# Hengle/AkariRender-1

Hardware: AMD Instinct MI355X
Metric: Msamples/sec (whole node), 10M-tri scene 1080p 1024spp, 1/2/4/8 MI355X (higher is better)
Workload: dtype f32; 1 GPU; C3 synthetic triangle soup (SURVEY.md §8d); triangles=10000002, width=1920, height=1080, spp=1025, max_depth=5, tile=64, parallelism=tile-split x1, bvh_leaf=4, builder=sbvh, form=k_path, ordered_fetch=True

## Files before the change

### akarirender-1_amd/akari_amd/capi.py

```python
from __future__ import annotations

import ctypes as C
import os
from pathlib import Path

import numpy as np

PKG_DIR = Path(__file__).resolve().parent.parent
PRODUCT_LIB = PKG_DIR / "libakr_hip.so"
EXPERIMENT_LIB_DIR = PKG_DIR.parent / "tools" / "experiments" / "lib"
LIB_PATH = Path(os.environ.get("AKR_HIP_LIB", PRODUCT_LIB))
if LIB_PATH != PRODUCT_LIB and LIB_PATH.resolve().parent != EXPERIMENT_LIB_DIR.resolve():
    raise ImportError(f"AKR_HIP_LIB={LIB_PATH}: only tools/experiments/lib/*.so may replace the product library")
GEN_PATH = PKG_DIR / "libakr_scenegen.so"


class AkrError(RuntimeError):
    """A non-zero status from the C-ABI (the reference's AKR_ASSERT_THROW convention)."""


class Ray(C.Structure):
    _fields_ = [("o", C.c_float * 3), ("tmin", C.c_float), ("d", C.c_float * 3), ("tmax", C.c_float)]


# ... 152 lines not shown
    "akr_hip_import_accel": (C.c_int, [_P, _P, C.c_uint64, _P, C.c_uint64, C.c_int32]),
    "akr_bvh_validate": (C.c_int, [_P, C.c_uint64, _P, C.c_uint64, C.c_uint64, C.POINTER(C.c_int32)]),
    "akr_hip_accel_info": (C.c_int, [_P, C.POINTER(AccelInfo)]),
    "akr_hip_accel_export": (C.c_int, [_P, _P, C.c_uint64, _P, C.c_uint64]),
    "akr_hip_set_camera": (C.c_int, [_P, C.POINTER(Camera)]),
    "akr_hip_set_lens": (C.c_int, [_P, C.c_float, C.c_float]),
    "akr_hip_lens": (C.c_int, [_P, C.POINTER(C.c_float), C.POINTER(C.c_float), C.POINTER(C.c_int32)]),
    "akr_hip_trace": (C.c_int, [_P, _P, C.c_uint64, _P, C.c_int]),
    "akr_hip_trace_device": (C.c_int, [_P, _P, C.c_uint64, _P, C.c_int, _P]),
    "akr_hip_render": (C.c_int, [_P, C.POINTER(PtParams), _P, C.c_int32, _P, _P]),
    "akr_hip_render_ao": (C.c_int, [_P, C.POINTER(AoParams), _P, C.c_int32, _P, _P]),
    "akr_hip_ray_steps": (C.c_int, [_P, _P, C.c_uint64]),
    "akr_hip_render_device": (C.c_int, [_P, C.POINTER(PtParams), _P, C.c_int32, _P, _P, _P,
                                        C.POINTER(C.c_uint64)]),
    "akr_hip_kernel_stats": (C.c_int, [_P, _P, C.c_int32, C.POINTER(C.c_int32)]),
    "akr_hip_trace_counts": (C.c_int, [_P, C.POINTER(TraceCounts)]),
    "akr_hip_path_profile": (C.c_int, [_P, C.POINTER(C.c_uint64), C.c_int32]),
    "akr_hip_reset_stats": (C.c_int, [_P]),
    "akr_hip_render_info": (C.c_int, [_P, C.POINTER(C.c_int32), C.POINTER(C.c_int32)]),
    "akr_hip_synchronize": (C.c_int, [_P]),
    "akr_hip_render_form": (C.c_int, [_P, C.POINTER(C.c_int32), C.POINTER(C.c_int32)]),
    "akr_hip_render_shading": (C.c_int, [_P, C.POINTER(C.c_int32)]),
    "akr_hip_render_form_inputs": (C.c_int, [_P, C.POINTER(C.c_int64), C.POINTER(C.c_int64), C.POINTER(C.c_int64)]),
    "akr_hip_pixel_probe": (C.c_int, [_P, _P, C.c_uint64]),
    "akr_bvh_host_build": (C.c_int, [_P, C.c_uint64, _P, C.c_uint64, C.POINTER(BuildParams), C.POINTER(_P),
                                     C.POINTER(AccelInfo)]),
    "akr_bvh_host_nodes": (_P, [_P]),
    "akr_bvh_host_tris": (_P, [_P]),
    "akr_bvh_host_free": (None, [_P]),
    "akr_hip_render_node": (C.c_int, [C.POINTER(_P), C.c_int32, C.POINTER(PtParams), _P, C.c_int32, _P, _P]),
    "akr_bvh_host_wide": (C.c_int, [_P, C.POINTER(C.c_uint64), C.POINTER(C.c_uint64), C.POINTER(C.c_uint32)]),
    "akr_bvh_host_wide_nodes": (_P, [_P]),
    "akr_bvh_host_wide_leaves": (_P, [_P]),
    "akr_hip_render_continue": (C.c_int, [_P, C.c_int32, _P, _P]),
    "akr_hip_render_continue_device": (C.c_int, [_P, C.c_int32, _P, _P, _P, C.POINTER(C.c_uint64)]),
    "akr_hip_render_state_info": (C.c_int, [_P, C.POINTER(RenderStateInfo)]),
    "akr_hip_render_state_export": (C.c_int, [_P, _P, _P, C.c_uint64]),
    "akr_hip_render_state_import": (C.c_int, [_P, C.POINTER(PtParams), _P, C.c_int32, _P, _P, C.c_uint64]),
    "akr_hip_render_continue_masked": (C.c_int, [_P, C.c_int32, _P, C.c_uint64, _P, _P]),
    "akr_hip_render_continue_masked_device": (C.c_int, [_P, C.c_int32, _P, C.c_uint64, _P, _P, _P,
                                                        C.POINTER(C.c_uint64)]),
    "akr_hip_render_state_spp_range": (C.c_int, [_P, C.POINTER(C.c_int32), C.POINTER(C.c_int32)]),
    "akr_hip_render_adaptive": (C.c_int, [_P, C.POINTER(PtParams), C.POINTER(AdaptiveParams), _P, C.c_int32, _P, _P,
                                          C.POINTER(AdaptiveInfo)]),
    "akr_hip_render_adaptive_device": (C.c_int, [_P, C.POINTER(PtParams), C.POINTER(AdaptiveParams), _P, C.c_int32,
                                                 _P, _P, _P, C.POINTER(C.c_uint64), C.POINTER(AdaptiveInfo)]),
    "akr_hip_adaptive_begin": (C.c_int, [_P, C.POINTER(PtParams), C.POINTER(AdaptiveParams), _P, C.c_int32,
                                         C.POINTER(AdaptiveInfo), C.POINTER(C.c_int32)]),
    "akr_hip_adaptive_step": (C.c_int, [_P, C.POINTER(AdaptiveInfo), C.POINTER(C.c_int32)]),
    "akr_hip_adaptive_error": (C.c_int, [_P, _P, _P, C.c_uint64]),
    "akr_hip_render_features": (C.c_int, [_P, C.POINTER(FeatureParams), _P, C.c_int32, _P]),
    "akr_hip_render_features_device": (C.c_int, [_P, C.POINTER(FeatureParams), _P, C.c_int32, _P, _P,
                                                 C.POINTER(C.c_uint64)]),
    "akr_hip_denoise": (C.c_int, [_P, C.POINTER(DenoiseParams), C.c_int32, C.c_int32, _P, _P, _P, _P]),
    "akr_hip_denoise_device": (C.c_int, [_P, C.POINTER(DenoiseParams), C.c_int32, C.c_int32, _P, _P, _P, _P, _P]),
    "akr_hip_render_variance": (C.c_int, [_P, _P]),
    "akr_hip_render_variance_device": (C.c_int, [_P, _P, _P, C.POINTER(C.c_uint64)]),
    "akr_hip_denoise_guided": (C.c_int, [_P, C.POINTER(DenoiseGuidedParams), C.c_int32, C.c_int32, _P, _P, _P, _P, _P]),
    "akr_hip_denoise_guided_device": (C.c_int, [_P, C.POINTER(DenoiseGuidedParams), C.c_int32, C.c_int32, _P, _P, _P, _P,
                                                _P, _P]),
}

_lib = None


def load_library() -> C.CDLL:
# ... 24 lines not shown
    lib = load_library()
    v = np.ascontiguousarray(vertices, np.float32).reshape(-1)
    i = np.ascontiguousarray(indices, np.int32).reshape(-1)
    p = BuildParams(max_leaf_size, n_bins, traversal_cost, intersect_cost, n_threads, builder, spatial_budget,
                    wide_collapse)
    h = C.c_void_p()
    info = AccelInfo()
    st = lib.akr_bvh_host_build(_ptr(v), v.size // 3, _ptr(i), i.size // 3, C.byref(p), C.byref(h), C.byref(info))
    if st != 0:
        raise AkrError("akr_bvh_host_build failed (invalid indices or build error)")
    try:
        nodes = np.empty(info.n_nodes, NODE_DTYPE)
        tris = np.empty(info.n_tris, TRI_DTYPE)
        C.memmove(nodes.ctypes.data, lib.akr_bvh_host_nodes(h), nodes.nbytes)
        if tris.nbytes:
            C.memmove(tris.ctypes.data, lib.akr_bvh_host_tris(h), tris.nbytes)
        if wide:
            nn, nl, root = C.c_uint64(0), C.c_uint64(0), C.c_uint32(0)
            if lib.akr_bvh_host_wide(h, C.byref(nn), C.byref(nl), C.byref(root)) != 0:
                raise AkrError("akr_bvh_host_wide failed")
            wn = np.empty(nn.value, NODE4_DTYPE)
            lv = np.empty(nl.value, LEAF_DTYPE)
            if wn.nbytes:
                C.memmove(wn.ctypes.data, lib.akr_bvh_host_wide_nodes(h), wn.nbytes)
            if lv.nbytes:
                C.memmove(lv.ctypes.data, lib.akr_bvh_host_wide_leaves(h), lv.nbytes)
    finally:
        lib.akr_bvh_host_free(h)
    if wide:
        return nodes, tris, info, (wn, lv, root.value)
    return nodes, tris, info


def validate_bvh(nodes, tris, n_scene_tris):
    nodes = np.ascontiguousarray(nodes, NODE_DTYPE)
    tris = np.ascontiguousarray(tris, TRI_DTYPE)
    d = C.c_int32(0)
    if load_library().akr_bvh_validate(_ptr(nodes), nodes.shape[0], _ptr(tris), tris.shape[0], int(n_scene_tris),
                                       C.byref(d)) != 0:
        raise AkrError("malformed BVH")
    return d.value


def render_node(ctxs, spp, max_depth, tiles, width, height, ray_clamp=0.0, exact_cull=False, radiance=None,
                weight=None, mis=None):
    lib = load_library()
    if mis is not None:
        for c in ctxs:
            c.set_option("mis", 1 if mis else 0)
    if radiance is None:
        radiance = np.zeros((height, width, 3), np.float32)
    if weight is None:
        weight = np.zeros((height, width), np.float32)
    assert radiance.dtype == np.float32 and radiance.flags.c_contiguous and radiance.size == 3 * width * height
    assert weight.dtype == np.float32 and weight.flags.c_contiguous and weight.size == width * height
    arr = (Rect * max(1, len(tiles)))(*[Rect(*t) for t in tiles])
    hs = (C.c_void_p * len(ctxs))(*[c.h for c in ctxs])
    p = PtParams(int(spp), int(max_depth), float(ray_clamp), PT_EXACT_CULL if exact_cull else 0)
    if lib.akr_hip_render_node(hs, len(ctxs), C.byref(p), _arr_ptr(arr), len(tiles), _ptr(radiance),
                               _ptr(weight)) != 0:
        raise AkrError(lib.akr_hip_last_error(ctxs[0].h).decode() if ctxs else "no contexts")
    return radiance, weight


def _ptr(a: np.ndarray):
    return a.ctypes.data_as(C.c_void_p)
# ... 487 lines not shown
```

### akarirender-1_amd/csrc/akr_device.h

```cpp
#pragma once
#include <stddef.h>
#include <stdint.h>
#include <hip/hip_runtime.h>
#include "../../include/akr_hip.h"
#include "../../include/akr_bvh_format.h"
#include "akr_path_forms.h"

#if defined(__HIP_DEVICE_COMPILE__)
#define AKR_GLOBAL __attribute__((address_space(1)))
#else
#define AKR_GLOBAL
#endif

namespace akr {

constexpr int kBlock = 256;
#ifndef AKR_TRACE_BLOCK
#define AKR_TRACE_BLOCK 256
#endif
constexpr int kTraceBlock = AKR_TRACE_BLOCK;
#ifndef AKR_STACK_LDS
#define AKR_STACK_LDS 15
#endif
#ifndef AKR_REFILL_MIN
// ... 34 lines not shown

__host__ __device__ inline uint32_t shard_begin(uint32_t n, uint32_t k) {
    return (uint32_t)(((uint64_t)n * k) / kWorkShards);
}

struct LightDev {
    float v[9];
    float tc[6];
    int32_t color_img;
    float Le[3];
    float area_half;
    float lng[3];
    float sel_pdf;
};

struct MatDev {
    int32_t type, double_sided, first, second;
    float color[3];
    int32_t color_img;
    float rough;
    int32_t rough_img;
    float frac;
    int32_t frac_img;
};
static_assert(sizeof(LightDev) == 96, "LightDev: six float4");

struct ShadeTri {
    float4 a;
    float4 b;
    float4 c;
    float4 d;
    float4 e;
};

struct TexDev {
    int32_t type;
    float value[3];
    int32_t w, h;
    int64_t off;
};

struct SceneDev {
    const AKR_GLOBAL ShadeTri *tri;
    const AKR_GLOBAL float *texcoords;
    int32_t has_image_tex;
    const AKR_GLOBAL MatDev *mats;
    const AKR_GLOBAL TexDev *texs;
    const AKR_GLOBAL float *images;
    const AKR_GLOBAL LightDev *lights;
    const AKR_GLOBAL float *light_cdf;
    int32_t n_lights;
    int32_t n_mats;
};

struct CameraDev {
    float r2c[16];
    float c2w[16];
    int32_t width, height;
};

struct TraceCounters {
    unsigned long long rays, box, tri;
    unsigned long long slots_trav, slots_leaf, slots_tri;
    unsigned long long visits;
    unsigned long long deep;
    unsigned long long leaves;
// ... 228 lines not shown
```

### akarirender-1_amd/csrc/bvh_build.h

```cpp
#pragma once
#include <stdint.h>
#include <exception>
#include <thread>
#include <vector>
#include "../../include/akr_hip.h"
#include "../../include/akr_bvh_format.h"

namespace akr {

template <class F>
void run_on_threads(int n, F &&f) {
    std::vector<std::exception_ptr> err((size_t)(n > 0 ? n : 0));
    auto call = [&](int k) {
        try {
            f(k);
        } catch (...) {
            err[(size_t)k] = std::current_exception();
        }
    };
    std::vector<std::thread> ts;
    std::vector<int> inline_k;
    for (int k = 1; k < n; k++) {
        try {
            ts.emplace_back(call, k);
// ... 9 lines not shown
}

struct BvhInput {
    const float *vertices;
    const int32_t *indices;
    uint64_t n_tris;
};

struct BvhOutput {
    std::vector<akr_bvh_node> nodes;
    std::vector<akr_bvh_tri> tris;
    int max_depth = 0;
    int max_leaf = 0;
    double sah_cost = 0;
    double build_ms = 0;
};

void build_bvh(const BvhInput &in, const akr_build_params &params, BvhOutput &out);

#ifdef __HIPCC__
void build_lbvh_gpu(const BvhInput &in, BvhOutput &out, hipStream_t st);
#endif

struct Bvh4Output {
    std::vector<akr_bvh4_node> nodes;
    std::vector<akr_bvh_leaf> leaves;
    uint32_t root_ref = AKR_CHILD_EMPTY;
    int max_depth = 0;
    float max_abs = 0.0f;
};

void build_bvh4(const std::vector<akr_bvh_node> &bvh2, Bvh4Output &out, int n_threads = 0, int collapse = 0);

int validate_bvh2(const akr_bvh_node *nodes, uint64_t n_nodes, const akr_bvh_tri *tris, uint64_t n_tris,
                  uint64_t n_scene_tris, int &max_leaf);

uint32_t quantize_lo(float bound, float origin, float s);
uint32_t quantize_hi(float bound, float origin, float s);

}
```

### akarirender-1_amd/csrc/bvh_wide.cpp

```cpp
#include <atomic>
#include <cmath>
#include <exception>
#include <thread>
#include <cstring>
#include <stdexcept>
#include "bvh_build.h"

namespace akr {

static bool real_le(uint32_t q, float s, float origin, float bound) {
    const long double v = (long double)origin + (long double)q * (long double)s;
    const long double m = std::ldexp(1.0L, -60) * (std::fabs((long double)origin) + 255.0L * s + std::fabs((long double)bound));
    return v + m <= (long double)bound;
}

static bool real_ge(uint32_t q, float s, float origin, float bound) {
    const long double v = (long double)origin + (long double)q * (long double)s;
    const long double m = std::ldexp(1.0L, -60) * (std::fabs((long double)origin) + 255.0L * s + std::fabs((long double)bound));
    return v - m >= (long double)bound;
}

namespace {

inline float pow2f(int k) { return std::ldexp(1.0f, k); }
// ... 298 lines not shown
                build(tasks[i], depth_of[w], abs_of[w], 0xffffffffu, no_spawn);
        });
        for (int w = 0; w < n_threads; w++) {
            max_depth = std::max(max_depth, depth_of[w]);
            max_abs = std::max(max_abs, abs_of[w]);
        }
        out.max_depth = max_depth;
        out.max_abs = max_abs;
    }
};

}

uint32_t quantize_lo(float bound, float origin, float s) {
    double q = std::floor(((double)bound - (double)origin) / (double)s);
    q = std::min(255.0, std::max(0.0, q));
    uint32_t qi = (uint32_t)q;
    while (qi > 0 && (std::fmaf((float)qi, s, origin) > bound || !real_le(qi, s, origin, bound))) qi--;
    if (std::fmaf((float)qi, s, origin) > bound || (qi > 0 && !real_le(qi, s, origin, bound)))
        throw std::runtime_error("quantize_lo: bound below origin");
    return qi;
}

uint32_t quantize_hi(float bound, float origin, float s) {
    double q = std::ceil(((double)bound - (double)origin) / (double)s);
    q = std::min(255.0, std::max(0.0, q));
    uint32_t qi = (uint32_t)q;
    while (qi < 255 && (std::fmaf((float)qi, s, origin) < bound || !real_ge(qi, s, origin, bound))) qi++;
    if (std::fmaf((float)qi, s, origin) < bound || !real_ge(qi, s, origin, bound))
        throw std::runtime_error("quantize_hi: bound beyond the frame");
    return qi;
}

int validate_bvh2(const akr_bvh_node *nodes, uint64_t n_nodes, const akr_bvh_tri *tris, uint64_t n_tris,
                  uint64_t n_scene_tris, int &max_leaf) {
    max_leaf = 0;
    if (n_nodes == 0) throw std::runtime_error("BVH: no nodes");
    if (n_nodes >= AKR_CHILD_LEAF) throw std::runtime_error("BVH: too many nodes");
    if (nodes[0].child[1] != AKR_CHILD_EMPTY) throw std::runtime_error("BVH: node 0 is not the virtual root");
    for (uint64_t t = 0; t < n_tris; t++)
        if (tris[t].gid >= n_scene_tris) throw std::runtime_error("BVH: triangle id beyond the scene");
    std::vector<uint8_t> seen(n_nodes, 0);
    std::vector<std::pair<uint32_t, int>> st;
    int depth = 0;
    auto child = [&](uint32_t r, int d) {
        if (r == AKR_CHILD_EMPTY) return;
        if (r & AKR_CHILD_LEAF) {
            const uint64_t first = akr_leaf_first(r), cnt = akr_leaf_count(r);
            if (cnt > AKR_LEAF_MAX || first + cnt > n_tris) throw std::runtime_error("BVH: leaf outside the triangles");
            if (d > AKR_BVH_MAX_DEPTH) throw std::runtime_error("BVH: deeper than AKR_BVH_MAX_DEPTH");
            max_leaf = std::max(max_leaf, (int)cnt);
            depth = std::max(depth, d);
            return;
        }
        if (r == 0 || r >= n_nodes) throw std::runtime_error("BVH: node reference out of range");
        if (seen[r]) throw std::runtime_error("BVH: a node is reached twice (not a tree)");
        seen[r] = 1;
        st.push_back({r, d});
    };
    seen[0] = 1;
    child(nodes[0].child[0], 1);
    while (!st.empty()) {
        const auto [n, d] = st.back();
        st.pop_back();
        if (d > AKR_BVH_MAX_DEPTH) throw std::runtime_error("BVH: deeper than AKR_BVH_MAX_DEPTH");
        depth = std::max(depth, d);
// ... 36 lines not shown
```

### akarirender-1_amd/csrc/capi.hip

```cpp
#include <hip/hip_runtime.h>

#include <algorithm>
#include <atomic>
#include <chrono>
#include <cmath>
#include <cstring>
#include <map>
#include <memory>
#include <stdexcept>
#include <string>
#include <thread>
#include <vector>

#include "akr_device.h"
#include "bvh_build.h"
#include "kernels.h"
#include "options.h"
#include "leaf_layout.h"
#include "path_plan.h"
#include "session.h"
#include "shade_simple.h"
#include "tile_layout.h"

using namespace akr;
// ... 420 lines not shown
            const akr_material &x = mats[m];
            auto tex_ok = [&](int32_t t) { return t >= 0 && t < (int32_t)texs.size(); };
            auto mat_ok = [&](int32_t t) { return t >= 0 && t < (int32_t)mats.size(); };
            bool ok = true;
            if (x.type == AKR_MAT_DIFFUSE || x.type == AKR_MAT_EMISSIVE) ok = tex_ok(x.color);
            else if (x.type == AKR_MAT_GLOSSY) ok = tex_ok(x.color) && tex_ok(x.roughness);
            else if (x.type == AKR_MAT_MIX) ok = tex_ok(x.fraction) && mat_ok(x.first) && mat_ok(x.second);
            else if (x.type == AKR_MAT_MIRROR) ok = tex_ok(x.color);
            else if (x.type == AKR_MAT_GLASS) ok = tex_ok(x.color) && tex_ok(x.roughness);
            else ok = false;
            if (!ok) throw std::runtime_error("material " + std::to_string(m) + " has an invalid type or reference");
            if (x.type == AKR_MAT_GLASS) {
                const akr_texture &t = texs[x.roughness];
                if (t.type != AKR_TEX_CONSTANT)
                    throw std::runtime_error("material " + std::to_string(m) +
                                             ": a Glass's index of refraction must be a constant texture, not an image");
                const float ior = t.value[0];
                if (!std::isfinite(ior) || ior < 1.0f || ior > 8.0f)
                    throw std::runtime_error("material " + std::to_string(m) +
                                             ": a Glass's index of refraction must be finite and lie in [1, 8]");
            }
        }
        has_specular = false;
        for (auto &m : mats) has_specular = has_specular || m.type == AKR_MAT_MIRROR || m.type == AKR_MAT_GLASS;
        simple_shading = true;
        for (auto &m : mats) simple_shading = simple_shading && (m.type == AKR_MAT_DIFFUSE || m.type == AKR_MAT_EMISSIVE);
        has_image_tex = false;
        for (auto &t : texs) {
            if (t.type == AKR_TEX_IMAGE && (t.image < 0 || t.image >= (int32_t)img_w.size()))
                throw std::runtime_error("image texture references a missing image");
            has_image_tex = has_image_tex || t.type == AKR_TEX_IMAGE;
        }
        simple_shading = simple_shading && !has_image_tex;
        std::vector<ShadeTri> st(nt);
        for (uint64_t g = 0; g < nt; g++) {
            const float *v0 = &verts[3 * (size_t)idx[3 * g + 0]];
            const float *v1 = &verts[3 * (size_t)idx[3 * g + 1]];
            const float *v2 = &verts[3 * (size_t)idx[3 * g + 2]];
            const float *nn = &normals[9 * g];
            float mbits;
            std::memcpy(&mbits, &matid[g], 4);
            st[g].a = make_float4(v0[0], v0[1], v0[2], mbits);
            st[g].b = make_float4(v1[0], v1[1], v1[2], nn[0]);
            st[g].c = make_float4(v2[0], v2[1], v2[2], nn[1]);
            st[g].d = make_float4(nn[2], nn[3], nn[4], nn[5]);
            st[g].e = make_float4(nn[6], nn[7], nn[8], 0.0f);
        }
        d_shade_tri.upload(st.data(), st.size(), stream);
        if (has_image_tex) d_tc.upload(texcoords.data(), texcoords.size(), stream);
        std::vector<MatDev> md(mats.size());
        for (size_t m = 0; m < mats.size(); m++) {
            const akr_material &x = mats[m];
            MatDev &d = md[m];
            std::memset(&d, 0, sizeof(d));
            akr::resolve_material(x, texs.data(), texs.size(), d);
        }
        d_mats.upload(md.data(), md.size(), stream);
        n_mats = (int32_t)md.size();
        std::vector<TexDev> td(texs.size());
        for (size_t k = 0; k < texs.size(); k++) {
            const akr_texture &t = texs[k];
            TexDev &d = td[k];
            std::memset(&d, 0, sizeof(d));
            d.type = t.type;
            for (int c = 0; c < 3; c++) d.value[c] = t.value[c];
            if (t.type == AKR_TEX_IMAGE) {
                d.w = img_w[t.image];
                d.h = img_h[t.image];
                d.off = img_off[t.image];
            }
        }
        d_texs.upload(td.data(), td.size(), stream);
        d_images.upload(images.data(), images.size(), stream);
        d_mesh_base.upload(mesh_base.data(), mesh_base.size(), stream);
        std::vector<LightDev> ld;
        for (auto &l : lights) {
            if (l.geom_id < 0 || l.geom_id + 1 >= (int32_t)mesh_base.size())
                throw std::runtime_error("light geom_id out of range");
            uint64_t g = (uint64_t)mesh_base[l.geom_id] + (uint64_t)l.prim_id;
// ... 961 lines not shown
    int c = 0;
    if (hipGetDeviceCount(&c) != hipSuccess) c = 0;
    *n = c;
    return 0;
}

int akr_hip_create(int device, akr_hip_ctx **out) {
    if (!out) return -1;
    *out = nullptr;
    int c = 0;
    if (hipGetDeviceCount(&c) != hipSuccess || device < 0 || device >= c) return -2;
    std::unique_ptr<akr_hip_ctx> ctx(new (std::nothrow) akr_hip_ctx());
    if (!ctx) return -1;
    ctx->device = device;
    if (hipSetDevice(device) != hipSuccess) return -1;
    if (hipStreamCreateWithFlags(&ctx->stream, hipStreamNonBlocking) != hipSuccess) return -1;
    if (hipEventCreateWithFlags(&ctx->ev_done, hipEventDisableTiming) != hipSuccess) return -1;
    hipDeviceProp_t prop;
    if (hipGetDeviceProperties(&prop, device) == hipSuccess && prop.multiProcessorCount > 0)
        ctx->n_cu = prop.multiProcessorCount;
    *out = ctx.release();
    return 0;
}

int akr_hip_destroy(akr_hip_ctx *ctx) {
    delete ctx;
    return 0;
}

const char *akr_hip_last_error(const akr_hip_ctx *ctx) { return ctx ? ctx->err.c_str() : "null context"; }

int akr_hip_set_option(akr_hip_ctx *ctx, const char *key, int64_t value) {
    return guard(ctx, [&] {
        const std::string why = set_option(ctx->opt, key, value);
        if (!why.empty()) throw std::runtime_error(why);
    });
}

int akr_hip_upload_mesh(akr_hip_ctx *ctx, const float *vertices, uint64_t n_vertices, const int32_t *indices,
                        const float *normals, const float *texcoords, const int32_t *material_indices,
                        uint64_t n_triangles, const int32_t *material_slots, int32_t n_slots, int32_t *geom_id) {
    return guard(ctx, [&] {
        if (n_triangles && (!vertices || !indices || !normals || !texcoords || !material_indices))
            throw std::runtime_error("null mesh array");
        if (ctx->n_tris() + n_triangles >= (1ull << 31)) throw std::runtime_error("scene too large");
        const uint64_t vb = ctx->verts.size() / 3;
        for (uint64_t i = 0; i < 3 * n_triangles; i++)
            if (indices[i] < 0 || (uint64_t)indices[i] >= n_vertices) throw std::runtime_error("vertex index out of range");
        for (uint64_t t = 0; t < n_triangles; t++) {
            int32_t m = material_indices[t];
            if (m >= n_slots) throw std::runtime_error("material index beyond the mesh's material list");
        }
        ctx->verts.insert(ctx->verts.end(), vertices, vertices + 3 * n_vertices);
        for (uint64_t i = 0; i < 3 * n_triangles; i++) ctx->idx.push_back((int32_t)(indices[i] + vb));
        ctx->normals.insert(ctx->normals.end(), normals, normals + 9 * n_triangles);
        ctx->texcoords.insert(ctx->texcoords.end(), texcoords, texcoords + 6 * n_triangles);
        for (uint64_t t = 0; t < n_triangles; t++) {
            int32_t m = material_indices[t];
            ctx->matid.push_back(m < 0 ? -1 : material_slots[m]);
        }
        if (geom_id) *geom_id = (int32_t)ctx->mesh_base.size() - 1;
        ctx->mesh_base.push_back((uint32_t)ctx->n_tris());
        ctx->scene_dirty = true;
        ctx->drop_session();
        ctx->accel_built = false;
    });
}

// ... 255 lines not shown
                h0.x = l.lo[0], h0.y = l.lo[1], h0.z = l.lo[2], h0.w = l.hi[0];
                uint32_t fc[2] = {l.first, l.count};
                h1.x = l.hi[1], h1.y = l.hi[2];
                std::memcpy(&h1.z, &fc[0], 4);
                std::memcpy(&h1.w, &fc[1], 4);
                o[0] = h0;
                o[1] = h1;
                std::memcpy(o + 2, tri4 + 3 * (size_t)l.first, sizeof(float4) * 3 * (size_t)l.count);
            }
            const size_t n0 = wn.size() * t / nt, n1 = wn.size() * (t + 1) / nt;
            for (size_t i = n0; i < n1; i++)
                for (auto &c : wn[i].child) c = remap(c);
        };
        run_on_threads(nt, fill);
        ctx->wide_root_dev = remap(ctx->bvh4.root_ref);
        size_t n_one = 0;
        for (const akr_bvh_leaf &l : leaves) n_one += l.count == 1 ? 1 : 0;
        ctx->leaf_one_kernel = akr::leaf_one_pays(n_one, leaves.size());
        ctx->d_wnodes.reserve(1);
        ctx->d_wleaves.reserve(1);
        ctx->d_wnodes.upload(wn.data(), wn.size(), ctx->stream);
        ctx->d_wleaves.upload(blob.get(), words + pad, ctx->stream);
        ctx->bvh_dev_bytes = (uint64_t)wn.size() * sizeof(akr_bvh4_node) + (uint64_t)(words + pad) * sizeof(float4);
        HIPCHK(hipStreamSynchronize(ctx->stream));
        ctx->d_tris.upload(reinterpret_cast<const float4 *>(b.tris.data()), 3 * b.tris.size(), ctx->stream);
        HIPCHK(hipStreamSynchronize(ctx->stream));
        ctx->info.n_nodes = b.nodes.size();
        ctx->info.n_tris = b.tris.size();
        ctx->info.max_depth = b.max_depth;
        ctx->info.max_leaf = b.max_leaf;
        ctx->info.build_ms = b.build_ms;
        ctx->info.sah_cost = b.sah_cost;
        ctx->accel_built = true;
        ctx->commit_scene();
}
}

int akr_hip_build_accel(akr_hip_ctx *ctx, const akr_build_params *params) {
    return guard(ctx, [&] {
        akr_build_params p{};
        p.max_leaf_size = 4;
        p.n_bins = 32;
        p.traversal_cost = 1.0f;
        p.intersect_cost = 4.0f;
        if (params) p = *params;
        BvhInput in{ctx->verts.data(), ctx->idx.data(), ctx->n_tris()};
        ctx->drop_session();
        ctx->accel_built = false;
        if (p.builder == AKR_BUILDER_LBVH) build_lbvh_gpu(in, ctx->bvh, ctx->stream);
        else if (p.builder == AKR_BUILDER_SAH || p.builder == AKR_BUILDER_SBVH) build_bvh(in, p, ctx->bvh);
        else throw std::runtime_error("unknown builder");
        if (p.wide_collapse != AKR_COLLAPSE_SAH && p.wide_collapse != AKR_COLLAPSE_BALANCED)
            throw std::runtime_error("unknown wide_collapse");
        ctx->wide_collapse = p.wide_collapse;
        finish_accel(ctx, p.n_threads);
    });
}

int akr_hip_import_accel(akr_hip_ctx *ctx, const void *nodes, uint64_t n_nodes, const void *tris, uint64_t n_tris,
                         int32_t n_threads) {
    return guard(ctx, [&] {
        if (!nodes || n_nodes == 0 || (n_tris && !tris)) throw std::runtime_error("null or empty BVH arrays");
        const auto *nd = reinterpret_cast<const akr_bvh_node *>(nodes);
        const auto *tr = reinterpret_cast<const akr_bvh_tri *>(tris);
        int max_leaf = 0;
        const int depth = validate_bvh2(nd, n_nodes, tr, n_tris, ctx->n_tris(), max_leaf);
// ... 754 lines not shown

int akr_bvh_validate(const void *nodes, uint64_t n_nodes, const void *tris, uint64_t n_tris, uint64_t n_scene_tris,
                     int32_t *max_depth) {
    try {
        if (!nodes || (n_tris && !tris)) return -1;
        int max_leaf = 0;
        const int d = validate_bvh2(reinterpret_cast<const akr_bvh_node *>(nodes), n_nodes,
                                    reinterpret_cast<const akr_bvh_tri *>(tris), n_tris, n_scene_tris, max_leaf);
        if (max_depth) *max_depth = d;
        return 0;
    } catch (...) {
        return -1;
    }
}

int akr_bvh_host_wide(akr_bvh_host *h, uint64_t *n_nodes, uint64_t *n_leaves, uint32_t *root_ref) {
    if (!h) return -1;
    try {
        if (!h->wide_built) {
            build_bvh4(h->out.nodes, h->wide, h->n_threads, h->collapse);
            h->wide_built = true;
        }
        if (n_nodes) *n_nodes = h->wide.nodes.size();
        if (n_leaves) *n_leaves = h->wide.leaves.size();
        if (root_ref) *root_ref = h->wide.root_ref;
        return 0;
    } catch (...) {
        return -1;
    }
}
const void *akr_bvh_host_wide_nodes(const akr_bvh_host *h) { return h ? h->wide.nodes.data() : nullptr; }
const void *akr_bvh_host_wide_leaves(const akr_bvh_host *h) { return h ? h->wide.leaves.data() : nullptr; }

int akr_hip_ray_steps(akr_hip_ctx *ctx, uint32_t *out, uint64_t n) {
    return guard(ctx, [&] {
        if (!ctx->opt.ray_steps || n > ctx->n_steps) throw std::runtime_error("no per-ray steps recorded for that many rays");
        if (n == 0) return;
        if (!out) throw std::runtime_error("null output");
        HIPCHK(hipMemcpyAsync(out, ctx->d_steps.p, n * sizeof(uint32_t), hipMemcpyDeviceToHost, ctx->stream));
        HIPCHK(hipStreamSynchronize(ctx->stream));
    });
}

int akr_hip_kernel_stats(akr_hip_ctx *ctx, akr_kernel_stat *out, int32_t max_n, int32_t *n) {
    return guard(ctx, [&] {
        ctx->flush_stats();
        int32_t k = 0;
        for (auto &kv : ctx->stat) {
            if (k < max_n && out) {
                akr_kernel_stat &s = out[k];
                std::memset(&s, 0, sizeof(s));
                std::strncpy(s.name, kv.first.c_str(), sizeof(s.name) - 1);
                s.launches = kv.second.launches;
                s.total_ms = kv.second.total;
                s.min_ms = kv.second.launches ? kv.second.mn : 0;
                s.max_ms = kv.second.mx;
            }
            k++;
        }
        if (n) *n = k;
    });
}

int akr_hip_trace_counts(akr_hip_ctx *ctx, akr_trace_counts *out) {
    return guard(ctx, [&] {
        std::memset(out, 0, sizeof(*out));
// ... 110 lines not shown
```

### akarirender-1_amd/csrc/kernels.hip

```cpp
#include "akr_device.h"
#include "akr_math.h"
#include "kernels.h"
#include "leaf_layout.h"

namespace akr {

__device__ __forceinline__ uint32_t fbits(float f) { return __float_as_uint(f); }
__device__ __forceinline__ float bitsf(uint32_t u) { return __uint_as_float(u); }

template <bool TIGHT, bool FAST = false>
__device__ __forceinline__ float box_test(float lox, float hix, float loy, float hiy, float loz, float hiz, V3 o,
                                          V3 invd, float tmin, float tmax) {
    float t0x = (lox - o.x) * invd.x, t1x = (hix - o.x) * invd.x;
    float t0y = (loy - o.y) * invd.y, t1y = (hiy - o.y) * invd.y;
    float t0z = (loz - o.z) * invd.z, t1z = (hiz - o.z) * invd.z;
    float m0, m1, t;
    if (FAST) {
        m0 = fmaxf(fmaxf(fminf(t0x, t1x), fminf(t0y, t1y)), fminf(t0z, t1z));
        m1 = fminf(fminf(fmaxf(t0x, t1x), fmaxf(t0y, t1y)), fmaxf(t0z, t1z));
        t = fmaxf(tmin, m0);
    } else {
        m0 = rmax(rmax(rmin(t0x, t1x), rmin(t0y, t1y)), rmin(t0z, t1z));
        m1 = rmin(rmin(rmax(t0x, t1x), rmax(t0y, t1y)), rmax(t0z, t1z));
        t = rmax(tmin, m0);
// ... 1953 lines not shown
    const unsigned long long st = wave_sum(c.strav), sl = wave_sum(c.sleaf), sr = wave_sum(c.stri);
    if (__lane_id() == 0) {
        atomicAdd(&a.counters[TRACE_CLOSEST].slots_trav, st);
        atomicAdd(&a.counters[TRACE_CLOSEST].slots_leaf, sl);
        atomicAdd(&a.counters[TRACE_CLOSEST].slots_tri, sr);
    }
}

template <bool COUNT>
__device__ __forceinline__ uint32_t probe_flags(const PathArgs &pa) {
    if (!COUNT) return AKR_PROBE_SEED;
    uint32_t f = AKR_PROBE_SEED | AKR_PROBE_RAYS;
    if (pa.probe_clock) f |= 4u | (uint32_t)((wall_clock64() >> 4) << 8);
    return f;
}

constexpr int kParkSlots = 8;

template <bool COUNT, bool TAB, bool ONE, bool SIMPLE, bool ENV = false>
__device__ __forceinline__ void path_plain(const PathArgs &pa, const EnvDev *env = nullptr) {
    if (pa.gate && *pa.gate != pa.gate_want) return;
    const TraceArgs &a = pa.t;
    __shared__ unsigned long long s_stack_mem[kStackLdsU64];
    __shared__ uint32_t s_park[kParkSlots][kTraceBlock];
    __shared__ uint4 s_tab[TAB ? kTabBytes / 16 : 1];
    lds_u64 *s_stack = (lds_u64 *)s_stack_mem;
    glb_u64 *stack_ovf = (glb_u64 *)a.stack_ovf;
    const uint32_t tid = threadIdx.x;
    const uint32_t gtid = blockIdx.x * kTraceBlock + tid;
    const uint32_t n = pa.n_pix;
    const int nb = pa.max_depth == 0 ? 1 : pa.max_depth;
    const bool ff = a.any_far_first != 0;
    const auto tab = PathTab<TAB>::make(pa.sc, s_tab);
    static_assert(kParkSlots >= 1 && kTraceBlock % 64 == 0, "the push's scratch words lie in a wave's park row 0");
    lds_u64 *dead = (lds_u64 *)&s_park[0][0] + (tid >> 1);
    PathCount c;
    if (COUNT) {
        c.lines = pa.lines;
        c.span[1] = pa.lines_span[1];
        c.span[2] = pa.lines_span[2];
        c.leaf_base = a.wide_leaves;
    }
    PixelFetch f{blockIdx.x % kWorkShards, 0, 0, (int)kWorkShards, n == 0};
    f.s_lo = shard_begin(n, f.shard);
    f.s_hi = shard_begin(n, f.shard + 1);

    uint32_t pix = 0, left = 0, seed = 0, pxr = 0;
    int depth = 0;
    V3 beta{1.0f, 1.0f, 1.0f}, Lr{0.0f, 0.0f, 0.0f}, scol{0.0f, 0.0f, 0.0f};
    float4 film = {0.0f, 0.0f, 0.0f, 0.0f};
    float4 pe0 = {}, pe1 = {};
    enum : uint32_t { F_BUSY = 1u, F_DONE = 2u, F_FIN = 4u, F_NEED = 8u, F_ANY = 16u, F_PEND = 32u };
    uint32_t fl = F_NEED;
    uint32_t pc_closest = 0, pc_shadow = 0;
    PathRay r{};
    r.best = kInf;
    r.bgid = kNoHit;
    r.cur = r.leaf = AKR_CHILD_EMPTY;
    unsigned long long p_outer = 0, p_procs = 0, p_tp = 0, p_tt = 0, p_tl = 0, p_lanes = 0, p_t0 = 0, p_t = 0, p_tsh = 0;
    unsigned long long p_tpark = 0, p_tnext = 0, p_tbegin = 0, p_tload = 0;
    if (COUNT) p_t0 = wall_clock64();

    while (true) {
        const unsigned long long waiting = mask_of((fl & (F_BUSY | F_DONE)) == 0);
        const uint32_t nwait = (uint32_t)__popcll(waiting);
        const uint32_t nbusy = (uint32_t)__popcll(mask_of((fl & F_BUSY) != 0));
        if (nwait == 0 && nbusy == 0) break;
        if (COUNT) {
            p_outer++;
            p_t = wall_clock64();
        }
        if (nwait > 0 && 64u * nwait >= pa.min_wait * (nwait + nbusy)) {
            if (COUNT) {
                p_procs++;
                p_lanes += nwait;
            }
            bool busy = (fl & F_BUSY) != 0, done = (fl & F_DONE) != 0, fin = (fl & F_FIN) != 0;
            bool need_pixel = (fl & F_NEED) != 0, any = (fl & F_ANY) != 0, pend = (fl & F_PEND) != 0;
            path_park(s_park, tid, r);
            __builtin_amdgcn_fence(__ATOMIC_RELEASE, "workgroup");
            asm volatile("" ::: "memory");
            bool fresh = false, next_any = false, sample_end = false, start = false;
            float4 ra = {}, rb = {};
            unsigned long long p_ts = 0;
            unsigned long long tl_phase = 0;
            if (COUNT) {
                p_ts = wall_clock64();
                p_tpark += p_ts - p_t;
            }
            if (!busy && !done && fin) {
                fin = false;
                const uint32_t hgid = r.bgid;
                [[maybe_unused]] const EnvDev *envp = env;
                if constexpr (ENV) {
                    unsigned long long eb = (unsigned long long)env;
                    asm volatile("" : "+s"(eb));
                    envp = (const EnvDev *)(const AKR_GLOBAL EnvDev *)eb;
                }
                if (any) {
                    if (hgid == kNoHit) {
                        Lr.x += scol.x;
                        Lr.y += scol.y;
                        Lr.z += scol.z;
                    }
                    if (pend) {
                        ra = pe0;
                        rb = pe1;
                        fresh = true;
                        pend = false;
                    } else {
                        sample_end = true;
                    }
                } else if (hgid == kNoHit) {
                    if constexpr (ENV) {
                        if (depth == 0) {
                            const V3 d{bitsf(s_park[3][tid]), bitsf(s_park[4][tid]), bitsf(s_park[5][tid])};
                            int ti, tj;
                            float len;
                            env_encode(envp->n, env_to_map(*envp, d), ti, tj, len);
                            const V3 e = mul(beta, env_lookup(*envp, ti, tj));
                            Lr.x += e.x;
                            Lr.y += e.y;
                            Lr.z += e.z;
                        }
                    }
                    sample_end = true;
                } else {
                    const V3 wo{-bitsf(s_park[3][tid]), -bitsf(s_park[4][tid]), -bitsf(s_park[5][tid])};
                    Bounce bo;
                    if (COUNT && pa.lines)
                        mark_lines(pa.lines, pa.lines_span[2], pa.lines_span[3], pa.sc.tri, pa.sc.tri + hgid,
                                   (uint32_t)sizeof(ShadeTri));
                    shade_hit_path<SIMPLE, ENV>(pa.sc, tab, hgid, r.bu, r.bv, wo, beta, seed, depth,
                                                pa.max_depth, depth == nb - 1, bo, COUNT ? &tl_phase : nullptr, envp);
                    if (bo.emit) {
                        Lr.x += bo.e.x;
                        Lr.y += bo.e.y;
                        Lr.z += bo.e.z;
                    }
                    if (bo.ext) {
                        beta = bo.nb;
                        depth++;
                    }
                    if (bo.sh) {
                        ra = bo.s0;
                        rb = bo.s1;
                        scol = bo.col;
                        next_any = true;
                        fresh = true;
                        pend = bo.ext;
                        pe0 = bo.e0;
                        pe1 = bo.e1;
                    } else if (bo.ext) {
                        ra = bo.e0;
                        rb = bo.e1;
                        fresh = true;
                    } else {
                        sample_end = true;
                    }
                }
            }
            if (COUNT) {
                const unsigned long long t = wall_clock64();
                p_tsh += t - p_ts;
                p_ts = t;
                p_tload += wave_max(tl_phase);
            }
            if (sample_end) {
                splat_one(film, make_float4(Lr.x, Lr.y, Lr.z, 0.0f), pa.ray_clamp);
                if (--left == 0) {
                    pa.film[pix] = film;
                    if (pa.state_out) pa.state_out[pix] = seed;
                    if (pa.probe)
                        pa.probe[pix] = make_uint4(seed, COUNT ? pc_closest : 0u, COUNT ? pc_shadow : 0u,
                                                   probe_flags<COUNT>(pa));
                    need_pixel = true;
                } else {
                    start = true;
                }
// ... 7 lines not shown
                if (pa.state_in) {
                    seed = pa.state_in[pix];
                    film = pa.film[pix];
                } else {
                    seed = (uint32_t)((int)(px & 0xFFFFu) + (int)(px >> 16) * pa.cam.width);
                    film = make_float4(0.0f, 0.0f, 0.0f, 0.0f);
                }
                start = true;
                if (COUNT) pc_closest = pc_shadow = 0;
            }
            if (start) {
                Lr = V3{0.0f, 0.0f, 0.0f};
                beta = V3{1.0f, 1.0f, 1.0f};
                depth = 0;
                const uint32_t px = pxr;
                camera_ray(pa.cam, (int)(px & 0xFFFFu), (int)(px >> 16), seed, ra, rb);
                fresh = true;
            }
            asm volatile("" ::: "memory");
            if (COUNT) {
                const unsigned long long t = wall_clock64();
                p_tnext += t - p_ts;
                p_ts = t;
            }
            path_unpark(s_park, tid, r, ff, any);
            if (fresh) {
                any = next_any;
                if (COUNT) {
                    pc_closest += any ? 0u : 1u;
                    pc_shadow += any ? 1u : 0u;
                }
                busy = path_begin<COUNT>(a, any, ra, rb, r, s_stack, stack_ovf, tid, gtid, c);
                fin = !busy;
            }
            fl = (busy ? F_BUSY : 0u) | (done ? F_DONE : 0u) | (fin ? F_FIN : 0u) | (need_pixel ? F_NEED : 0u) |
                 (any ? F_ANY : 0u) | (pend ? F_PEND : 0u);
            asm("" : "+v"(fl));
            if (COUNT) p_tbegin += wall_clock64() - p_ts;
        }
        if (COUNT) {
            const unsigned long long t = wall_clock64();
            p_tp += t - p_t;
            p_t = t;
        }
        const unsigned long long bm = mask_of((fl & F_BUSY) != 0);
        if (bm == 0) continue;
        const bool busy = in_mask(bm);
        [[maybe_unused]] const int kd = (fl & F_ANY) != 0 ? 1 : 0;
        if constexpr (COUNT)
            path_traverse<COUNT, kWhileExitPath, true>(busy, kd, r, a.wide_nodes, s_stack, stack_ovf, a.ovf_threads, tid,
                                                       gtid, c, pa.pop_keep, pa.pop_rounds, dead);
        else
            path_traverse_masks<kWhileExitPath>(bm, r, a.wide_nodes, s_stack, stack_ovf, a.ovf_threads, tid, gtid,
                                                pa.pop_keep, pa.pop_rounds, dead);
        if (COUNT) {
            const unsigned long long t = wall_clock64();
            p_tt += t - p_t;
            p_t = t;
        }
        bool ended;
        if constexpr (COUNT || !ONE) {
            const bool hit_any = path_leaf<COUNT>(busy, kd, r, a.wide_leaves, c);
            ended = busy && (hit_any || r.cur == AKR_CHILD_EMPTY);
        } else {
            const unsigned long long hm = path_leaf_masks(bm, mask_of((fl & F_ANY) != 0), r, a.wide_leaves);
            ended = in_mask(bm & (hm | mask_of(r.cur == AKR_CHILD_EMPTY)));
// ... 1380 lines not shown
```

### akarirender-1_amd/csrc/options.h

```cpp
#pragma once
#include <stdint.h>
#include <string.h>

#include <string>

namespace akr {

struct Options {
    bool verify = true;
    int pixel_probe = 0;
    bool probe() const { return pixel_probe != 0; }
    bool probe_clock() const { return pixel_probe == 2; }
    bool fault_test = false;
    bool film_variance = false;
    bool mis = false;
    bool env_path = false;
    bool env_forms = false;

    int path_defer = 2;
    int path_spec = 2;
    int64_t path_tail_ppl10 = 60;
    int path_tail_steps = 12;
    int64_t path_cache_mb = 128;
    int64_t path_spec_pixels = 0;
    int64_t path_defer_pixels = 0;
    int64_t path_defer_min_tris = 0;
    int path_spec_fetch = 3;
    int64_t path_spec_fetch_pixels = 0;
    int path_spec_depth = 3;
    bool path_mix = true;
    bool path_tab = true;
    int path_order = 2;
    int path_order_pair = 2;
    int path_prio = 0;
    int path_order_min_spp = 16;
    int64_t path_order_share_pixels = 1200000;
    int path_order_share_min_spp = 16;
    int path_order_shift = 2;
    int path_order_classes = 16;
    int path_order_cap = 64;
    int path_order_sub = 0;
    int path_order_pilot_spp = 0;
    bool wave_order = true;
    int path_kernel = 2;
    int64_t path_auto_pixels = INT64_MAX;
    bool path_auto_complex = false;
    bool serial_shadow = false;
    bool any_far_first = false;
    int path_min_wait = 0;
    int path_pop_rounds = 2, path_pop_keep = 4;
// ... 77 lines not shown
    {"verify", &Options::verify},
    {"rays_per_lane", &Options::rays_per_lane, 1, 64},
};

inline const OptionRow *find_option(const char *key) {
    for (const OptionRow &r : kOptionTable)
        if (key && strcmp(r.name, key) == 0) return &r;
    return nullptr;
}

inline int64_t get_option(const Options &o, const OptionRow &r) { return r.b ? (o.*r.b ? 1 : 0) : (r.i ? o.*r.i : o.*r.l); }

inline std::string set_option(Options &o, const char *key, int64_t value) {
    if (key && strcmp(key, "film_variance") == 0) {
        if (value != 0 && value != 1) return "film_variance must be in [0, 1]";
        o.film_variance = value == 1;
        return {};
    }
    if (key && strcmp(key, "mis") == 0) {
        if (value != 0 && value != 1) return "mis must be in [0, 1]";
        o.mis = value == 1;
        return {};
    }
    if (key && strcmp(key, "env_path") == 0) {
        if (value != 0 && value != 1) return "env_path must be in [0, 1]";
        o.env_path = value == 1;
        return {};
    }
    if (key && strcmp(key, "env_forms") == 0) {
        if (value != 0 && value != 1) return "env_forms must be in [0, 1]";
        o.env_forms = value == 1;
        return {};
    }
    const OptionRow *r = find_option(key);
    if (!r) return "unknown option '" + std::string(key ? key : "") + "'";
    const bool pow2 = r->kind == OptionRow::POW2;
    if (value < r->lo || value > r->hi || (pow2 && (value & (value - 1)) != 0))
        return std::string(key) + " must be in [" + std::to_string(r->lo) + ", " + std::to_string(r->hi) + "]" +
               (pow2 ? " and a power of two" : "");
    if (r->kind == OptionRow::FLAG) o.*r->b = value != 0;
    else if (r->kind == OptionRow::TRI) o.*r->i = value == 2 ? 2 : (value != 0 ? 1 : 0);
    else if (r->l) o.*r->l = value;
    else o.*r->i = (int)(value < INT32_MAX ? value : INT32_MAX);
    return {};
}

}
```

### include/akr_hip.h

```cpp
#ifndef AKR_HIP_H
#define AKR_HIP_H

#include <stdint.h>

#ifdef __cplusplus
extern "C" {
#endif

#define AKR_HIP_API_VERSION 3

typedef struct akr_hip_ctx akr_hip_ctx;

typedef struct akr_ray {
    float o[3];
    float tmin;
    float d[3];
    float tmax;
} akr_ray;

typedef struct akr_hit {
    float t;
    float u, v;
    int32_t geom_id;
    int32_t prim_id;
// ... 230 lines not shown
int akr_hip_denoise(akr_hip_ctx *ctx, const akr_denoise_params *params, int32_t width, int32_t height,
                    const float *radiance, const float *weight, const float *features, float *out_rgb);
int akr_hip_denoise_device(akr_hip_ctx *ctx, const akr_denoise_params *params, int32_t width, int32_t height,
                           const float *d_radiance, const float *d_weight, const float *d_features,
                           float *d_out_rgb, void *stream);

int akr_hip_render_variance(akr_hip_ctx *ctx, float *variance);
int akr_hip_render_variance_device(akr_hip_ctx *ctx, float *d_variance, void *stream, uint64_t *n_pixels);

typedef struct akr_denoise_guided_params {
    akr_denoise_params base;
    float sigma_variance;
    int32_t _pad[3];
} akr_denoise_guided_params;
int akr_hip_denoise_guided(akr_hip_ctx *ctx, const akr_denoise_guided_params *params, int32_t width, int32_t height,
                           const float *radiance, const float *weight, const float *features, const float *variance,
                           float *out_rgb);
int akr_hip_denoise_guided_device(akr_hip_ctx *ctx, const akr_denoise_guided_params *params, int32_t width,
                                  int32_t height, const float *d_radiance, const float *d_weight,
                                  const float *d_features, const float *d_variance, float *d_out_rgb, void *stream);

typedef struct akr_bvh_host akr_bvh_host;
int akr_bvh_host_build(const float *vertices, uint64_t n_vertices, const int32_t *indices,
                       uint64_t n_triangles, const akr_build_params *params, akr_bvh_host **out,
                       akr_accel_info *info);
const void *akr_bvh_host_nodes(const akr_bvh_host *h);
const void *akr_bvh_host_tris(const akr_bvh_host *h);
void akr_bvh_host_free(akr_bvh_host *h);
int akr_bvh_host_wide(akr_bvh_host *h, uint64_t *n_nodes, uint64_t *n_leaves, uint32_t *root_ref);
int akr_bvh_validate(const void *nodes, uint64_t n_nodes, const void *tris, uint64_t n_tris,
                     uint64_t n_scene_tris, int32_t *max_depth);
const void *akr_bvh_host_wide_nodes(const akr_bvh_host *h);
const void *akr_bvh_host_wide_leaves(const akr_bvh_host *h);

int akr_hip_kernel_stats(akr_hip_ctx *ctx, akr_kernel_stat *out, int32_t max_n, int32_t *n);
int akr_hip_trace_counts(akr_hip_ctx *ctx, akr_trace_counts *out);

int akr_hip_path_profile(akr_hip_ctx *ctx, uint64_t *out, int32_t n);
int akr_hip_reset_stats(akr_hip_ctx *ctx);
int akr_hip_render_info(akr_hip_ctx *ctx, int32_t *lanes, int32_t *passes);
#define AKR_FORM_NONE (-1)
#define AKR_FORM_WAVEFRONT 0
#define AKR_FORM_PATH 2
#define AKR_FORM_PATH_DEFER 3
#define AKR_FORM_PATH_SPEC 4
int akr_hip_render_form(akr_hip_ctx *ctx, int32_t *form, int32_t *ordered);
#define AKR_SHADING_NONE (-1)
#define AKR_SHADING_GENERAL 0
#define AKR_SHADING_SIMPLE 1
int akr_hip_render_shading(akr_hip_ctx *ctx, int32_t *shading);
int akr_hip_render_form_inputs(akr_hip_ctx *ctx, int64_t *pixels_per_lane_x1000, int64_t *pilot_rays,
                               int64_t *pilot_steps);
int akr_hip_synchronize(akr_hip_ctx *ctx);
int akr_hip_pixel_probe(akr_hip_ctx *ctx, akr_pixel_probe *out, uint64_t n);
int akr_hip_ray_steps(akr_hip_ctx *ctx, uint32_t *out, uint64_t n);

#ifdef __cplusplus
}
#endif
#endif
```

Before: 621.9 Msamples/s.

## Start shadow-ray traversal at a precomputed BVH subtree near the hit triangle

Adds a per-triangle entry-node table built on the host: the deepest wide-BVH ancestor that holds at least a threshold number of leaves. The table is packed into the spare lane of each ShadeTri. In the path kernel, shadow/any-hit rays push the normal start node onto the stack and begin traversal at that local subtree. Nearby occluders can then be found earlier and the any-hit traversal cut short. If no local occluder exists, the subtree is visited again through the root, which costs extra work. It also adds host table-building time and one extra field read per hit.

```diff
diff --git a/akarirender-1_amd/akari_amd/capi.py b/akarirender-1_amd/akari_amd/capi.py
--- a/akarirender-1_amd/akari_amd/capi.py
+++ b/akarirender-1_amd/akari_amd/capi.py
@@ -208,6 +208,7 @@
     "akr_bvh_host_wide": (C.c_int, [_P, C.POINTER(C.c_uint64), C.POINTER(C.c_uint64), C.POINTER(C.c_uint32)]),
     "akr_bvh_host_wide_nodes": (_P, [_P]),
     "akr_bvh_host_wide_leaves": (_P, [_P]),
+    "akr_bvh_shadow_entry": (C.c_int, [_P, C.c_uint64, _P, C.c_uint64, _P, C.c_uint64, C.c_uint64, C.c_uint32, _P]),
     "akr_hip_render_continue": (C.c_int, [_P, C.c_int32, _P, _P]),
     "akr_hip_render_continue_device": (C.c_int, [_P, C.c_int32, _P, _P, _P, C.POINTER(C.c_uint64)]),
     "akr_hip_render_state_info": (C.c_int, [_P, C.POINTER(RenderStateInfo)]),
@@ -298,6 +299,17 @@
     return nodes, tris, info
 
 
+def shadow_entry_table(wide_nodes, leaves, tris, n_scene_tris, min_leaves):
+    wn = np.ascontiguousarray(wide_nodes, NODE4_DTYPE)
+    lv = np.ascontiguousarray(leaves, LEAF_DTYPE)
+    tr = np.ascontiguousarray(tris, TRI_DTYPE)
+    out = np.zeros(int(n_scene_tris), np.uint32)
+    if load_library().akr_bvh_shadow_entry(_ptr(wn), wn.shape[0], _ptr(lv), lv.shape[0], _ptr(tr), tr.shape[0],
+                                           int(n_scene_tris), int(min_leaves), _ptr(out)) != 0:
+        raise AkrError("akr_bvh_shadow_entry failed (malformed wide view)")
+    return out
+
+
 def validate_bvh(nodes, tris, n_scene_tris):
     nodes = np.ascontiguousarray(nodes, NODE_DTYPE)
     tris = np.ascontiguousarray(tris, TRI_DTYPE)
diff --git a/akarirender-1_amd/csrc/akr_device.h b/akarirender-1_amd/csrc/akr_device.h
--- a/akarirender-1_amd/csrc/akr_device.h
+++ b/akarirender-1_amd/csrc/akr_device.h
@@ -90,6 +90,7 @@
     float4 d;
     float4 e;
 };
+constexpr uint32_t kShadowEntryNone = 0xFFFFFFFFu;
 
 struct TexDev {
     int32_t type;
diff --git a/akarirender-1_amd/csrc/bvh_build.h b/akarirender-1_amd/csrc/bvh_build.h
--- a/akarirender-1_amd/csrc/bvh_build.h
+++ b/akarirender-1_amd/csrc/bvh_build.h
@@ -65,6 +65,10 @@
 
 void build_bvh4(const std::vector<akr_bvh_node> &bvh2, Bvh4Output &out, int n_threads = 0, int collapse = 0);
 
+void shadow_entry_table(const akr_bvh4_node *nodes, uint64_t n_nodes, const akr_bvh_leaf *leaves, uint64_t n_leaves,
+                        const akr_bvh_tri *tris, uint64_t n_tris, uint64_t n_scene_tris, uint32_t min_leaves,
+                        uint32_t *out);
+
 int validate_bvh2(const akr_bvh_node *nodes, uint64_t n_nodes, const akr_bvh_tri *tris, uint64_t n_tris,
                   uint64_t n_scene_tris, int &max_leaf);
 
diff --git a/akarirender-1_amd/csrc/bvh_wide.cpp b/akarirender-1_amd/csrc/bvh_wide.cpp
--- a/akarirender-1_amd/csrc/bvh_wide.cpp
+++ b/akarirender-1_amd/csrc/bvh_wide.cpp
@@ -354,6 +354,44 @@
     return qi;
 }
 
+void shadow_entry_table(const akr_bvh4_node *nodes, uint64_t n_nodes, const akr_bvh_leaf *leaves, uint64_t n_leaves,
+                        const akr_bvh_tri *tris, uint64_t n_tris, uint64_t n_scene_tris, uint32_t min_leaves,
+                        uint32_t *out) {
+    for (uint64_t g = 0; g < n_scene_tris; g++) out[g] = 0;
+    if (n_nodes == 0) return;
+    if (n_nodes >= AKR_CHILD_LEAF) throw std::runtime_error("shadow_entry_table: too many wide nodes");
+    std::vector<uint32_t> below(n_nodes), entry(n_nodes, 0);
+    for (uint64_t i = n_nodes; i-- > 0;) {
+        uint64_t nl = 0;
+        for (uint32_t c : nodes[i].child) {
+            if (c == AKR_CHILD_EMPTY) continue;
+            if (c & AKR_CHILD_LEAF) {
+                if ((c & 0x7FFFFFFFu) >= n_leaves) throw std::runtime_error("shadow_entry_table: leaf reference out of range");
+                nl++;
+            } else {
+                if (c <= i || c >= n_nodes) throw std::runtime_error("shadow_entry_table: wide nodes are not in preorder");
+                nl += below[c];
+            }
+        }
+        below[i] = (uint32_t)std::min<uint64_t>(nl, 0xFFFFFFFFull);
+    }
+    for (uint64_t i = 0; i < n_nodes; i++)
+        for (uint32_t c : nodes[i].child) {
+            if (c == AKR_CHILD_EMPTY) continue;
+            if (!(c & AKR_CHILD_LEAF)) {
+                entry[c] = below[c] >= min_leaves ? c : entry[i];
+                continue;
+            }
+            const akr_bvh_leaf &l = leaves[c & 0x7FFFFFFFu];
+            if ((uint64_t)l.first + l.count > n_tris) throw std::runtime_error("shadow_entry_table: leaf outside the triangles");
+            for (uint32_t k = 0; k < l.count; k++) {
+                const uint32_t gid = tris[(uint64_t)l.first + k].gid;
+                if (gid >= n_scene_tris) throw std::runtime_error("shadow_entry_table: triangle id beyond the scene");
+                out[gid] = entry[i];
+            }
+        }
+}
+
 int validate_bvh2(const akr_bvh_node *nodes, uint64_t n_nodes, const akr_bvh_tri *tris, uint64_t n_tris,
                   uint64_t n_scene_tris, int &max_leaf) {
     max_leaf = 0;
diff --git a/akarirender-1_amd/csrc/capi.hip b/akarirender-1_amd/csrc/capi.hip
--- a/akarirender-1_amd/csrc/capi.hip
+++ b/akarirender-1_amd/csrc/capi.hip
@@ -476,6 +476,12 @@
             has_image_tex = has_image_tex || t.type == AKR_TEX_IMAGE;
         }
         simple_shading = simple_shading && !has_image_tex;
+        std::vector<uint32_t> entry;
+        if (opt.shadow_entry > 0 && accel_built && bvh4.root_ref == 0 && !bvh4.nodes.empty()) {
+            entry.resize(nt);
+            akr::shadow_entry_table(bvh4.nodes.data(), bvh4.nodes.size(), bvh4.leaves.data(), bvh4.leaves.size(),
+                                    bvh.tris.data(), bvh.tris.size(), nt, (uint32_t)opt.shadow_entry, entry.data());
+        }
         std::vector<ShadeTri> st(nt);
         for (uint64_t g = 0; g < nt; g++) {
             const float *v0 = &verts[3 * (size_t)idx[3 * g + 0]];
@@ -488,7 +494,10 @@
             st[g].b = make_float4(v1[0], v1[1], v1[2], nn[0]);
             st[g].c = make_float4(v2[0], v2[1], v2[2], nn[1]);
             st[g].d = make_float4(nn[2], nn[3], nn[4], nn[5]);
-            st[g].e = make_float4(nn[6], nn[7], nn[8], 0.0f);
+            const uint32_t ebits = entry.empty() || entry[g] == 0 ? kShadowEntryNone : entry[g];
+            float ew;
+            std::memcpy(&ew, &ebits, 4);
+            st[g].e = make_float4(nn[6], nn[7], nn[8], ew);
         }
         d_shade_tri.upload(st.data(), st.size(), stream);
         if (has_image_tex) d_tc.upload(texcoords.data(), texcoords.size(), stream);
@@ -1516,8 +1525,10 @@
 
 int akr_hip_set_option(akr_hip_ctx *ctx, const char *key, int64_t value) {
     return guard(ctx, [&] {
+        const int64_t entry_was = ctx->opt.shadow_entry;
         const std::string why = set_option(ctx->opt, key, value);
         if (!why.empty()) throw std::runtime_error(why);
+        if (ctx->opt.shadow_entry != entry_was) ctx->scene_dirty = true;
     });
 }
 
@@ -1839,6 +1850,7 @@
         ctx->info.build_ms = b.build_ms;
         ctx->info.sah_cost = b.sah_cost;
         ctx->accel_built = true;
+        if (ctx->opt.shadow_entry > 0) ctx->scene_dirty = true;
         ctx->commit_scene();
 }
 }
@@ -2659,6 +2671,19 @@
 const void *akr_bvh_host_wide_nodes(const akr_bvh_host *h) { return h ? h->wide.nodes.data() : nullptr; }
 const void *akr_bvh_host_wide_leaves(const akr_bvh_host *h) { return h ? h->wide.leaves.data() : nullptr; }
 
+int akr_bvh_shadow_entry(const void *wide_nodes, uint64_t n_nodes, const void *leaves, uint64_t n_leaves, const void *tris,
+                         uint64_t n_tris, uint64_t n_scene_tris, uint32_t min_leaves, uint32_t *out) {
+    try {
+        if ((n_nodes && !wide_nodes) || (n_leaves && !leaves) || (n_tris && !tris) || (n_scene_tris && !out)) return -1;
+        akr::shadow_entry_table(reinterpret_cast<const akr_bvh4_node *>(wide_nodes), n_nodes,
+                                reinterpret_cast<const akr_bvh_leaf *>(leaves), n_leaves,
+                                reinterpret_cast<const akr_bvh_tri *>(tris), n_tris, n_scene_tris, min_leaves, out);
+        return 0;
+    } catch (...) {
+        return -1;
+    }
+}
+
 int akr_hip_ray_steps(akr_hip_ctx *ctx, uint32_t *out, uint64_t n) {
     return guard(ctx, [&] {
         if (!ctx->opt.ray_steps || n > ctx->n_steps) throw std::runtime_error("no per-ray steps recorded for that many rays");
diff --git a/akarirender-1_amd/csrc/kernels.hip b/akarirender-1_amd/csrc/kernels.hip
--- a/akarirender-1_amd/csrc/kernels.hip
+++ b/akarirender-1_amd/csrc/kernels.hip
@@ -2009,6 +2009,7 @@
     const int nb = pa.max_depth == 0 ? 1 : pa.max_depth;
     const bool ff = a.any_far_first != 0;
     const auto tab = PathTab<TAB>::make(pa.sc, s_tab);
+    constexpr bool kEntry = SIMPLE || COUNT;
     static_assert(kParkSlots >= 1 && kTraceBlock % 64 == 0, "the push's scratch words lie in a wave's park row 0");
     lds_u64 *dead = (lds_u64 *)&s_park[0][0] + (tid >> 1);
     PathCount c;
@@ -2059,6 +2060,7 @@
             asm volatile("" ::: "memory");
             bool fresh = false, next_any = false, sample_end = false, start = false;
             float4 ra = {}, rb = {};
+            uint32_t entry = kShadowEntryNone;
             unsigned long long p_ts = 0;
             unsigned long long tl_phase = 0;
             if (COUNT) {
@@ -2108,6 +2110,8 @@
                     if (COUNT && pa.lines)
                         mark_lines(pa.lines, pa.lines_span[2], pa.lines_span[3], pa.sc.tri, pa.sc.tri + hgid,
                                    (uint32_t)sizeof(ShadeTri));
+                    uint32_t hit_entry = kShadowEntryNone;
+                    if constexpr (kEntry) hit_entry = fbits(pa.sc.tri[hgid].e.w);
                     shade_hit_path<SIMPLE, ENV>(pa.sc, tab, hgid, r.bu, r.bv, wo, beta, seed, depth,
                                                 pa.max_depth, depth == nb - 1, bo, COUNT ? &tl_phase : nullptr, envp);
                     if (bo.emit) {
@@ -2122,6 +2126,7 @@
                     if (bo.sh) {
                         ra = bo.s0;
                         rb = bo.s1;
+                        entry = hit_entry;
                         scol = bo.col;
                         next_any = true;
                         fresh = true;
@@ -2195,6 +2200,13 @@
                 }
                 busy = path_begin<COUNT>(a, any, ra, rb, r, s_stack, stack_ovf, tid, gtid, c);
                 fin = !busy;
+                if constexpr (kEntry) {
+                    if (busy && entry != kShadowEntryNone && r.cur != AKR_CHILD_EMPTY) {
+                        lds_put(s_stack, 0, tid, (unsigned long long)r.cur);
+                        r.sp = 1;
+                        r.cur = entry;
+                    }
+                }
             }
             fl = (busy ? F_BUSY : 0u) | (done ? F_DONE : 0u) | (fin ? F_FIN : 0u) | (need_pixel ? F_NEED : 0u) |
                  (any ? F_ANY : 0u) | (pend ? F_PEND : 0u);
diff --git a/akarirender-1_amd/csrc/options.h b/akarirender-1_amd/csrc/options.h
--- a/akarirender-1_amd/csrc/options.h
+++ b/akarirender-1_amd/csrc/options.h
@@ -5,6 +5,9 @@
 #include <string>
 
 namespace akr {
+
+constexpr int64_t kShadowEntryDefault = 4096;
+constexpr int64_t kShadowEntryMax = int64_t(1) << 30;
 
 struct Options {
     bool verify = true;
@@ -16,6 +19,7 @@
     bool mis = false;
     bool env_path = false;
     bool env_forms = false;
+    int64_t shadow_entry = kShadowEntryDefault;
 
     int path_defer = 2;
     int path_spec = 2;
@@ -159,6 +163,11 @@
         o.env_forms = value == 1;
         return {};
     }
+    if (key && strcmp(key, "shadow_entry") == 0) {
+        if (value < 0 || value > kShadowEntryMax) return "shadow_entry must be in [0, " + std::to_string(kShadowEntryMax) + "]";
+        o.shadow_entry = value;
+        return {};
+    }
     const OptionRow *r = find_option(key);
     if (!r) return "unknown option '" + std::string(key ? key : "") + "'";
     const bool pow2 = r->kind == OptionRow::POW2;
diff --git a/include/akr_hip.h b/include/akr_hip.h
--- a/include/akr_hip.h
+++ b/include/akr_hip.h
@@ -286,6 +286,9 @@
                      uint64_t n_scene_tris, int32_t *max_depth);
 const void *akr_bvh_host_wide_nodes(const akr_bvh_host *h);
 const void *akr_bvh_host_wide_leaves(const akr_bvh_host *h);
+int akr_bvh_shadow_entry(const void *wide_nodes, uint64_t n_nodes, const void *leaves, uint64_t n_leaves,
+                         const void *tris, uint64_t n_tris, uint64_t n_scene_tris, uint32_t min_leaves,
+                         uint32_t *out);
 
 int akr_hip_kernel_stats(akr_hip_ctx *ctx, akr_kernel_stat *out, int32_t max_n, int32_t *n);
 int akr_hip_trace_counts(akr_hip_ctx *ctx, akr_trace_counts *out);
```

Result: no change. 627.9 Msamples/s (median of 6 runs) (+1.0%).
